# ilkyyldz95/3DmedicalImageSegmentation

Measured on AMD Instinct MI355X. Metric: training volumes/sec (96^3, 4-class), higher is better.
Workload: dtype bf16; 1 GPU; UNETR(img=96^3,patch=16,hidden=768,layers=12,heads=12,classes=4) fwd+DiceCE+bwd+AdamW, batch 2/GPU, configs[1]; global_batch=2

## Files before the change

### 3dmedicalimagesegmentation_amd/csrc/gemm_bf16.hip

```cpp
#include <type_traits>
#include "gemm_kernel.hpp"

namespace {

typedef __attribute__((address_space(3))) void lds_void_t;
typedef const __attribute__((address_space(1))) void gbl_void_t;
typedef short s16x4 __attribute__((ext_vector_type(4)));
typedef short s16x8 __attribute__((ext_vector_type(8)));
#define LDS_AS_ __attribute__((address_space(3)))

struct EpBf {
    int vec_ok;
    float* C; long ldc;
    uint16_t* Cb; long ldcb;
    const float* bias;
    const float* res; long ldr; int res_mod;
    float* pre;
    const float* aux; long ldaux;
    int act, accumulate; float alpha;
    int tc_d, tc_h, tc_w, tc_cout;
    __device__ __forceinline__ long tc_off(int m, int n) const {
        const int tap = n / tc_cout, co = n - tap * tc_cout;
        const int x = m % tc_w; int t = m / tc_w; const int y = t % tc_h; t /= tc_h; const int z = t % tc_d; const int b = t / tc_d;
        const long ov = (((long)b * 2 * tc_d + 2 * z + (tap >> 2)) * 2 * tc_h + 2 * y + ((tap >> 1) & 1)) * 2 * tc_w + 2 * x + (tap & 1);
        return ov * ldcb + co;
    }
    __device__ __forceinline__ void store(int, int m, int n, float v) const {
        v *= alpha;
        if (bias) v += bias[n];
        if (pre) pre[(long)m * ldc + n] = v;
        if (act == 1) v = gelu_fast(v);
        else if (act == 2) v *= gelu_grad_fast(aux[(long)m * ldaux + n]);
        if (res) v += res[(long)(m % res_mod) * ldr + n];
        if (C) {
            if (accumulate) v += C[(long)m * ldc + n];
            C[(long)m * ldc + n] = v;
        }
        if (Cb) {
            __bf16 h = (__bf16)v;
            Cb[tc_cout ? tc_off(m, n) : (long)m * ldcb + n] = __builtin_bit_cast(uint16_t, h);
        }
    }
    __device__ __forceinline__ void store4(int m, int n, f32x4 v) const {
        v *= alpha;
        if (bias) v += *(const f32x4*)(bias + n);
        if (pre) *(f32x4*)(pre + (long)m * ldc + n) = v;
        if (act == 1) {
#pragma unroll
            for (int e = 0; e < 4; ++e) v[e] = gelu_fast(v[e]);
        } else if (act == 2) {
            const f32x4 a = *(const f32x4*)(aux + (long)m * ldaux + n);
#pragma unroll
            for (int e = 0; e < 4; ++e) v[e] *= gelu_grad_fast(a[e]);
        }
        if (res) v += *(const f32x4*)(res + (long)(m % res_mod) * ldr + n);
        if (C) {
            if (accumulate) v += *(const f32x4*)(C + (long)m * ldc + n);
            *(f32x4*)(C + (long)m * ldc + n) = v;
        }
        if (Cb) *(bf16x4*)(Cb + (tc_cout ? tc_off(m, n) : (long)m * ldcb + n)) = __builtin_convertvector(v, bf16x4);
    }
    struct Ops { f32x4 b, a, r, c; };
    __device__ __forceinline__ Ops load4(int m, int n) const {
        Ops o;
        const f32x4 z = {0.f, 0.f, 0.f, 0.f};
        o.b = bias ? *(const f32x4*)(bias + n) : z;
        o.a = act == 2 ? *(const f32x4*)(aux + (long)m * ldaux + n) : z;
        o.r = res ? *(const f32x4*)(res + (long)(m % res_mod) * ldr + n) : z;
        o.c = (C && accumulate) ? *(const f32x4*)(C + (long)m * ldc + n) : z;
        return o;
    }
    __device__ __forceinline__ void finish4(int m, int n, f32x4 v, const Ops& o) const {
        v *= alpha;
        if (bias) v += o.b;
        if (pre) *(f32x4*)(pre + (long)m * ldc + n) = v;
        if (act == 1) {
#pragma unroll
            for (int e = 0; e < 4; ++e) v[e] = gelu_fast(v[e]);
        } else if (act == 2) {
#pragma unroll
            for (int e = 0; e < 4; ++e) v[e] *= gelu_grad_fast(o.a[e]);
        }
        if (res) v += o.r;
        if (C) {
            if (accumulate) v += o.c;
            *(f32x4*)(C + (long)m * ldc + n) = v;
        }
        if (Cb) *(bf16x4*)(Cb + (tc_cout ? tc_off(m, n) : (long)m * ldcb + n)) = __builtin_convertvector(v, bf16x4);
    }
};

template <int CPR> __device__ __forceinline__ int bkn_x(int r) {
    if constexpr (CPR >= 16) return ((r & 3) | (((r >> 3) & 1) << 2)) << 1;
    else return (((r >> 1) & 1) | (((r >> 3) & 1) << 1)) << 1;
}

__device__ __forceinline__ bool tile_of(int L, int mt, int nt, int& tm, int& tn) {
    const int T = mt * nt, per = (T + 7) >> 3;
    const int t = (L & 7) * per + (L >> 3);
    if ((L >> 3) >= per || t >= T) return false;
    tm = t % mt; tn = t / mt;
    return true;
}

template <int WM, int WN, int WVM, int WVN, bool BKN, int NS, int X3 = 0>
__global__ void __launch_bounds__(64 * WVM * WVN)
gemm_bf16_kernel(int M, int N, int K, int mt, int nt, int splits, int kper,
                 const typename std::conditional<X3 != 0, float, uint16_t>::type* __restrict__ A, long lda,
                 const typename std::conditional<X3 != 0, float, uint16_t>::type* __restrict__ B, long ldb, EpBf ep,
                 float* __restrict__ ws) {
    typedef typename std::conditional<X3 != 0, float, uint16_t>::type ET;
    constexpr int ESZ = sizeof(ET), CE = 16 / ESZ;
    constexpr int NT = 64 * WVM * WVN, BM = 16 * WM * WVM, BN = 16 * WN * WVN, BK = 128 / ESZ;
    constexpr int A_BYTES = BM * 128;
    constexpr int B_BYTES = BKN ? BK * BN * ESZ : BN * 128;
    static_assert(!(X3 != 0 && BKN) || BN >= 64, "the [K,N] fp32 image needs >= 16 chunks per row for its swizzle");
    constexpr int STAGE = A_BYTES + B_BYTES;
    constexpr int AIT = A_BYTES / 16 / NT, BIT = B_BYTES / 16 / NT;
    static_assert(A_BYTES % (16 * NT) == 0 && B_BYTES % (16 * NT) == 0, "tile must divide into whole wave DMAs");
    constexpr int G = AIT + BIT;
    static_assert(NS >= 2 && (NS - 2) * G <= 63, "vmcnt is a 6-bit counter");
    __shared__ __attribute__((aligned(1024))) char lds[NS * STAGE];

    int tm, tn;
    if (!tile_of(blockIdx.x, mt, nt, tm, tn)) return;
    const int m0 = tm * BM, n0 = tn * BN;
    const int split = blockIdx.y, kbeg = split * kper, kend = min(K, kbeg + kper);
    const int nk = (kend - kbeg) / BK;
    const int tid = threadIdx.x, lane = tid & 63;
    const int wave = __builtin_amdgcn_readfirstlane(tid >> 6), wm = wave / WVN, wn = wave % WVN;

    const ET* asrc[AIT];
    const ET* bsrc[BIT];
#pragma unroll
    for (int i = 0; i < AIT; ++i) {
        const int id = tid + i * NT, r = id >> 3, c = (id & 7) ^ ((r >> 1) & 7);
        asrc[i] = A + (long)min(m0 + r, M - 1) * lda + kbeg + c * CE;
    }
#pragma unroll
    for (int i = 0; i < BIT; ++i) {
        const int id = tid + i * NT;
        if constexpr (!BKN) {
            const int r = id >> 3, c = (id & 7) ^ ((r >> 1) & 7);
            bsrc[i] = B + (long)min(n0 + r, N - 1) * ldb + kbeg + c * CE;
        } else {
            constexpr int CPR = BN / CE;
            const int r = id / CPR, s = id % CPR;
            const int c = X3 != 0 ? (s ^ (((r >> 2) & 3) << 2)) : (s ^ bkn_x<CPR>(r));
            bsrc[i] = B + (long)(kbeg + r) * ldb + min(n0 + c * CE, N - CE);
        }
    }
    auto issue = [&](int kt, int buf) {
        char* la = lds + buf * STAGE;
        char* lb = la + A_BYTES;
#pragma unroll
        for (int i = 0; i < AIT; ++i)
            __builtin_amdgcn_global_load_lds((gbl_void_t*)(asrc[i] + (long)kt * BK), (lds_void_t*)(la + (wave * 64 + i * NT) * 16), 16, 0, 0);
#pragma unroll
        for (int i = 0; i < BIT; ++i) {
            const ET* g = BKN ? bsrc[i] + (long)kt * BK * ldb : bsrc[i] + (long)kt * BK;
            __builtin_amdgcn_global_load_lds((gbl_void_t*)g, (lds_void_t*)(lb + (wave * 64 + i * NT) * 16), 16, 0, 0);
        }
    };

    f32x4 acc[WM][WN];
#pragma unroll
    for (int i = 0; i < WM; ++i)
#pragma unroll
        for (int j = 0; j < WN; ++j) acc[i][j] = (f32x4){0.f, 0.f, 0.f, 0.f};

#pragma unroll
    for (int s = 0; s < NS - 1; ++s)
        if (s < nk) issue(s, s);
    for (int kt = 0; kt < nk; ++kt) {
        if (kt + NS - 2 < nk) asm volatile("s_waitcnt vmcnt(%0) lgkmcnt(0)\n\ts_barrier" ::"n"((NS - 2) * G) : "memory");
        else asm volatile("s_waitcnt vmcnt(0) lgkmcnt(0)\n\ts_barrier" ::: "memory");
        if (kt + NS - 1 < nk) issue(kt + NS - 1, (kt + NS - 1) % NS);
        const char* la = lds + (kt % NS) * STAGE;
        const char* lb = la + A_BYTES;
        u32x4 a[2][WM], b[2][WN];
#pragma unroll
        for (int kb = 0; kb < 2; ++kb) {
#pragma unroll
            for (int i = 0; i < WM; ++i)
                a[kb][i] = *(const u32x4*)(la + lds_tile_off((wm * WM + i) * 16 + (lane & 15), kb * 4 + (lane >> 4)));
#pragma unroll
            for (int j = 0; j < WN; ++j) {
                if constexpr (!BKN) {
                    b[kb][j] = *(const u32x4*)(lb + lds_tile_off((wn * WN + j) * 16 + (lane & 15), kb * 4 + (lane >> 4)));
                } else if constexpr (X3 != 0) {
                    const int col = (wn * WN + j) * 16 + (lane & 15), g = lane >> 4;
                    const char* pb = lb + (kb * 16 + 4 * g) * (BN * 4) + ((((col >> 2) ^ (g << 2))) << 4) + (col & 3) * 4;
#pragma unroll
                    for (int t = 0; t < 4; ++t) b[kb][j][t] = *(const uint32_t*)(pb + t * (BN * 4));
                } else {
                    constexpr int CPR = BN / 8;
                    const int cc = lane & 15, g = lane >> 4, q = cc >> 2, p = cc & 3;
                    const int r0 = kb * 32 + 8 * g + q, r1 = r0 + 4;
                    const int ch = (wn * WN + j) * 2 + (p >> 1);
                    const int s0 = ch ^ bkn_x<CPR>(r0);
                    const int s1 = ch ^ bkn_x<CPR>(r1);
                    s16x4 lo = __builtin_amdgcn_ds_read_tr16_b64_v4i16((LDS_AS_ s16x4*)(lb + r0 * (BN * 2) + s0 * 16 + (p & 1) * 8));
                    s16x4 hi = __builtin_amdgcn_ds_read_tr16_b64_v4i16((LDS_AS_ s16x4*)(lb + r1 * (BN * 2) + s1 * 16 + (p & 1) * 8));
                    s16x8 v = {lo[0], lo[1], lo[2], lo[3], hi[0], hi[1], hi[2], hi[3]};
                    b[kb][j] = __builtin_bit_cast(u32x4, v);
                }
            }
        }
        __builtin_amdgcn_sched_barrier(0);
#pragma unroll
        for (int kb = 0; kb < 2; ++kb) {
            if constexpr (X3 == 2) {
                u32x4 ah[WM], al[WM];
#pragma unroll
                for (int i = 0; i < WM; ++i) x3_dup(a[kb][i], ah[i], al[i]);
#pragma unroll
                for (int i = 0; i < WM; ++i)
#pragma unroll
                    for (int j = 0; j < WN; ++j) {
                        PrecBF16::mma(acc[i][j], b[kb][j], ah[i]);
                        PrecBF16::mma(acc[i][j], b[kb][j], al[i]);
                    }
            } else if constexpr (X3 == 1) {
                u32x4 bh[WN], bl[WN];
#pragma unroll
                for (int i = 0; i < WM; ++i) a[kb][i] = x3_words(a[kb][i]);
#pragma unroll
                for (int j = 0; j < WN; ++j) x3_dup(b[kb][j], bh[j], bl[j]);
#pragma unroll
                for (int i = 0; i < WM; ++i)
#pragma unroll
                    for (int j = 0; j < WN; ++j) {
                        PrecBF16::mma(acc[i][j], bh[j], a[kb][i]);
                        PrecBF16::mma(acc[i][j], bl[j], a[kb][i]);
                    }
            } else {
#pragma unroll
                for (int i = 0; i < WM; ++i)
#pragma unroll
                    for (int j = 0; j < WN; ++j) PrecBF16::mma(acc[i][j], b[kb][j], a[kb][i]);
            }
        }
        __builtin_amdgcn_sched_barrier(0);
    }

    const bool vec4 = ep.vec_ok;
    if (vec4 && splits == 1) {
        constexpr int RB = WM * WN <= 4 ? WM : 1;
#pragma unroll
        for (int i0 = 0; i0 < WM; i0 += RB) {
            EpBf::Ops ops[RB][WN];
#pragma unroll
            for (int i = 0; i < RB; ++i)
#pragma unroll
                for (int j = 0; j < WN; ++j) {
                    const int m = min(m0 + (wm * WM + i0 + i) * 16 + (lane & 15), M - 1);
                    const int n = min(n0 + (wn * WN + j) * 16 + 4 * (lane >> 4), N - 4);
                    ops[i][j] = ep.load4(m, n);
                }
#pragma unroll
            for (int i = 0; i < RB; ++i)
#pragma unroll
                for (int j = 0; j < WN; ++j) {
                    const int m = m0 + (wm * WM + i0 + i) * 16 + (lane & 15);
                    const int n = n0 + (wn * WN + j) * 16 + 4 * (lane >> 4);
                    if (m < M && n < N) ep.finish4(m, n, acc[i0 + i][j], ops[i][j]);
                }
        }
        return;
    }
#pragma unroll
    for (int i = 0; i < WM; ++i)
#pragma unroll
        for (int j = 0; j < WN; ++j) {
            const int m = m0 + (wm * WM + i) * 16 + (lane & 15);
            const int n = n0 + (wn * WN + j) * 16 + 4 * (lane >> 4);
            if (m >= M || n >= N) continue;
            if (vec4) {
                if (splits > 1) *(f32x4*)(ws + ((long)split * M + m) * N + n) = acc[i][j];
                else ep.store4(m, n, acc[i][j]);
            } else {
#pragma unroll
                for (int r = 0; r < 4; ++r)
                    if (n + r < N) {
                        if (splits > 1) ws[((long)split * M + m) * N + n + r] = acc[i][j][r];
                        else ep.store(0, m, n + r, acc[i][j][r]);
                    }
            }
        }
}

template <int WM, int WN, int WVM, int WVN, bool BKN, int NS, int X3 = 0>
int launch_bf16(int M, int N, int K, const typename std::conditional<X3 != 0, float, uint16_t>::type* A, long lda,
                const typename std::conditional<X3 != 0, float, uint16_t>::type* B, long ldb, const EpBf& ep,
                float* ws, size_t ws_bytes, hipStream_t st, int* partial_splits = nullptr) {
    constexpr int BM = 16 * WM * WVM, BN = 16 * WN * WVN, BKE = X3 != 0 ? 32 : 64;
    const int mt = cdiv(M, BM), nt = cdiv(N, BN), ksteps = K / BKE;
    const long tiles = (long)mt * nt;
    int splits = 1;
    const int min_steps = X3 != 0 ? 48 : 24;
    if (tiles < 192 && ksteps >= min_steps) splits = std::min(ksteps / (min_steps / 2), (int)((512 + tiles - 1) / tiles));
    if (const char* e = getenv("UNETR_GEMM_SPLITS")) { int v = atoi(e); if (v > 0) splits = std::min(v, ksteps); }
    while (splits > 1 && (size_t)splits * M * N * sizeof(float) > ws_bytes) --splits;
    if (splits < 1 || ws == nullptr) splits = 1;
    const int kper = cdiv(ksteps, splits) * BKE;
    splits = cdiv(K, kper);
    const int per = cdiv(tiles, 8);
    hipLaunchKernelGGL((gemm_bf16_kernel<WM, WN, WVM, WVN, BKN, NS, X3>), dim3(per * 8, splits), dim3(64 * WVM * WVN), 0, st,
                       M, N, K, mt, nt, splits, kper, A, lda, B, ldb, ep, ws);
    if (partial_splits) *partial_splits = splits;
    if (splits > 1 && !partial_splits)
        hipLaunchKernelGGL((splitk_reduce_kernel<EpBf, false>), dim3(cdiv(N, 64), cdiv(M, 4), 1), dim3(256), 0, st, M, N, splits, ws, ep);
    return unetr_check_launch();
}

template <int BUF>
struct BufC { static constexpr int value = BUF; };

template <int WN>
__device__ __forceinline__ void big_epilogue(f32x4 (&acc)[8][WN], const EpBf& ep, char* lds, int M, int N, int m0, int n0,
                                             int wave, int lane, int wr, int wc) {
    const int mb = m0 + wr * 128 + (lane & 15), nb = n0 + wc * (16 * WN) + 4 * (lane >> 4);
    if (!ep.vec_ok) {
        for (int t = 0; t < 8 * WN; ++t) {
            const int i = t / WN, j = t - i * WN, m = mb + i * 16, n = nb + j * 16;
            f32x4 v = (f32x4){0.f, 0.f, 0.f, 0.f};
#pragma clang loop unroll(full)
            for (int ii = 0; ii < 8; ++ii)
#pragma clang loop unroll(full)
                for (int jj = 0; jj < WN; ++jj) v = (ii == i && jj == j) ? acc[ii][jj] : v;
            if (m < M)
                for (int r = 0; r < 4; ++r)
                    if (n + r < N) ep.store(0, m, n + r, v[r]);
        }
        return;
    }
    const int kind = (ep.act == 1 ? 1 : ep.act == 2 ? 2 : 0);
    char* const stg = lds + wave * 16384;
    const int rr = lane >> 4, rc = lane & 15;
    const int ncol = n0 + wc * (16 * WN) + rc * 4;
    const bool cok = rc < 4 * WN && ncol < N;
    f32x4 bias4 = (f32x4){0.f, 0.f, 0.f, 0.f};
    if (ep.bias && cok) bias4 = *(const f32x4*)(ep.bias + ncol);
    auto half = [&](auto kc, auto hc) __attribute__((always_inline)) {
        constexpr int KIND = decltype(kc)::value, h = decltype(hc)::value;
#pragma clang loop unroll(full)
        for (int i = 0; i < 4; ++i)
#pragma clang loop unroll(full)
            for (int j = 0; j < WN; ++j) {
                const int r = i * 16 + (lane & 15), ch = j * 4 + (lane >> 4);
                *(f32x4*)(stg + r * 256 + ((ch ^ (r & 7)) << 4)) = acc[h * 4 + i][j] * ep.alpha;
            }
        asm volatile("s_waitcnt lgkmcnt(0)" ::: "memory");
#pragma clang loop unroll(full)
        for (int it = 0; it < 16; ++it) {
            const int r = it * 4 + rr, m = m0 + wr * 128 + h * 64 + r;
            f32x4 v = *(const f32x4*)(stg + r * 256 + ((rc ^ (r & 7)) << 4)) + bias4;
            if (m < M && cok) {
                if (ep.pre) *(f32x4*)(ep.pre + (long)m * ep.ldc + ncol) = v;
                if constexpr (KIND == 1) {
#pragma unroll
                    for (int e = 0; e < 4; ++e) v[e] = gelu_fast(v[e]);
                } else if constexpr (KIND == 2) {
                    const f32x4 a = *(const f32x4*)(ep.aux + (long)m * ep.ldaux + ncol);
#pragma unroll
                    for (int e = 0; e < 4; ++e) v[e] *= gelu_grad_fast(a[e]);
                }
                if (ep.res) v += *(const f32x4*)(ep.res + (long)(m % ep.res_mod) * ep.ldr + ncol);
                if (ep.C) {
                    if (ep.accumulate) v += *(const f32x4*)(ep.C + (long)m * ep.ldc + ncol);
                    *(f32x4*)(ep.C + (long)m * ep.ldc + ncol) = v;
                }
                if (ep.Cb) *(bf16x4*)(ep.Cb + (long)m * ep.ldcb + ncol) = __builtin_convertvector(v, bf16x4);
            }
        }
        asm volatile("s_waitcnt lgkmcnt(0)" ::: "memory");
    };
    if (kind == 1) { half(BufC<1>{}, BufC<0>{}); half(BufC<1>{}, BufC<1>{}); }
    else if (kind == 2) { half(BufC<2>{}, BufC<0>{}); half(BufC<2>{}, BufC<1>{}); }
    else { half(BufC<0>{}, BufC<0>{}); half(BufC<0>{}, BufC<1>{}); }
}

template <int WN>
__global__ void __launch_bounds__(512, 2)
gemm_bf16_big_kernel(int M, int N, int K, int mt, int nt, int n_fast,
                     const uint16_t* __restrict__ A, long lda, const uint16_t* __restrict__ B, long ldb, EpBf ep) {
    constexpr int NT = 512, HALF = 128 * 128, BN = 64 * WN, BUFB = 2 * HALF + BN * 128;
    constexpr int LDSB = 2 * BUFB > 8 * 16384 ? 2 * BUFB : 8 * 16384;
    __shared__ __attribute__((aligned(1024))) char lds[LDSB];

    int tm, tn;
    {
        const int T = mt * nt, per = (T + 7) >> 3, L = blockIdx.x;
        const int t = (L & 7) * per + (L >> 3);
        if ((L >> 3) >= per || t >= T) return;
        if (n_fast) { tn = t % nt; tm = t / nt; } else { tm = t % mt; tn = t / mt; }
    }
    const int m0 = tm * 256, n0 = tn * BN;
    const int nk = K / 64;
    const int tid = threadIdx.x, lane = tid & 63;
    const int wave = __builtin_amdgcn_readfirstlane(tid >> 6), wr = wave >> 2, wc = wave & 3;

    const uint16_t* asrc[2][2];
    const uint16_t* bsrc[WN];
#pragma unroll
    for (int h = 0; h < 2; ++h)
#pragma unroll
        for (int i = 0; i < 2; ++i) {
            const int id = tid + i * NT, r = id >> 3, c = (id & 7) ^ ((r >> 1) & 7);
            asrc[h][i] = A + (long)min(m0 + h * 128 + r, M - 1) * lda + c * 8;
        }
#pragma unroll
    for (int i = 0; i < WN; ++i) {
        const int id = tid + i * NT, r = id >> 3, c = (id & 7) ^ ((r >> 1) & 7);
        bsrc[i] = B + (long)min(n0 + r, N - 1) * ldb + c * 8;
    }
    auto dma = [&](const uint16_t* const (&src)[2], int T, char* dst) __attribute__((always_inline)) {
#pragma unroll
        for (int i = 0; i < 2; ++i)
            __builtin_amdgcn_global_load_lds((gbl_void_t*)(src[i] + (long)T * 64), (lds_void_t*)(dst + (wave * 64 + i * NT) * 16), 16, 0, 0);
    };
    auto dmab = [&](int T, char* dst) __attribute__((always_inline)) {
#pragma unroll
        for (int i = 0; i < WN; ++i)
            __builtin_amdgcn_global_load_lds((gbl_void_t*)(bsrc[i] + (long)T * 64), (lds_void_t*)(dst + (wave * 64 + i * NT) * 16), 16, 0, 0);
    };
    int off[2];
#pragma unroll
    for (int kh = 0; kh < 2; ++kh) off[kh] = lds_tile_off(lane & 15, kh * 4 + (lane >> 4));

    f32x4 acc[8][WN];
#pragma unroll
    for (int i = 0; i < 8; ++i)
#pragma unroll
        for (int j = 0; j < WN; ++j) acc[i][j] = (f32x4){0.f, 0.f, 0.f, 0.f};
    u32x4 af[4][2], bf[WN][2];
    dma(asrc[0], 0, lds);
    dma(asrc[1], 0, lds + HALF);
    dmab(0, lds + 2 * HALF);
    if (nk > 1) {
        dmab(1, lds + BUFB + 2 * HALF);
        asm volatile("s_waitcnt vmcnt(%0)\n\ts_barrier" ::"n"(WN) : "memory");
    } else {
        asm volatile("s_waitcnt vmcnt(0)\n\ts_barrier" ::: "memory");
    }
    if (wr == 1) asm volatile("s_barrier" ::: "memory");
    __builtin_amdgcn_sched_barrier(0);

#define BIG_MEM_END() do { asm volatile("s_waitcnt lgkmcnt(0)\n\ts_barrier" ::: "memory"); __builtin_amdgcn_sched_barrier(0); } while (0)
#define BIG_CMP_END(last_) do { __builtin_amdgcn_sched_barrier(0); if (!(last_)) asm volatile("s_barrier" ::: "memory"); __builtin_amdgcn_sched_barrier(0); } while (0)
#define BIG_HALF(qa_) do {                                                                           \
        __builtin_amdgcn_s_setprio(1);                                                               \
        _Pragma("unroll") for (int kh = 0; kh < 2; ++kh)                                             \
            _Pragma("unroll") for (int i = 0; i < 4; ++i)                                            \
                _Pragma("unroll") for (int j = 0; j < WN; ++j)                                       \
                    PrecBF16::mma(acc[(qa_) * 4 + i][j], bf[j][kh], af[i][kh]);                      \
        __builtin_amdgcn_s_setprio(0);                                                               \
    } while (0)

    auto ktile = [&](int T, auto bufc) __attribute__((always_inline)) {
        constexpr int b = decltype(bufc)::value;
        char* const cur = lds + b * BUFB;
        char* const oth = lds + (b ^ 1) * BUFB;
        const char* la = cur + wr * HALF;
        const char* lb = cur + 2 * HALF + wc * (16 * WN) * 128;
        const bool n1 = T + 1 < nk, n2 = T + 2 < nk;
        {
#pragma unroll
            for (int kh = 0; kh < 2; ++kh) {
#pragma unroll
                for (int j = 0; j < WN; ++j) bf[j][kh] = *(const u32x4*)(lb + off[kh] + j * 2048);
            }
            __builtin_amdgcn_sched_barrier(0);
#pragma unroll
            for (int kh = 0; kh < 2; ++kh) {
#pragma unroll
                for (int i = 0; i < 4; ++i) af[i][kh] = *(const u32x4*)(la + off[kh] + i * 2048);
            }
            if (n1) { dma(asrc[0], T + 1, oth); dma(asrc[1], T + 1, oth + HALF); }
            BIG_MEM_END();
            BIG_HALF(0);
            BIG_CMP_END(false);
#pragma unroll
            for (int kh = 0; kh < 2; ++kh) {
#pragma unroll
                for (int i = 0; i < 4; ++i) af[i][kh] = *(const u32x4*)(la + off[kh] + (4 + i) * 2048);
            }
            if (n2) {
                dmab(T + 2, cur + 2 * HALF);
                asm volatile("s_waitcnt vmcnt(%0)" ::"n"(WN) : "memory");
            } else if (n1) {
                asm volatile("s_waitcnt vmcnt(0)" ::: "memory");
            }
            BIG_MEM_END();
            BIG_HALF(1);
            BIG_CMP_END(!n1 && wr == 1);
        }
    };
    for (int T = 0; T < nk; T += 2) {
        ktile(T, BufC<0>{});
        if (T + 1 < nk) ktile(T + 1, BufC<1>{});
    }
#undef BIG_MEM_END
#undef BIG_CMP_END
#undef BIG_HALF

    big_epilogue<WN>(acc, ep, lds, M, N, m0, n0, wave, lane, wr, wc);
}

static int launch_bf16_big(int M, int N, int K, const uint16_t* A, long lda, const uint16_t* B, long ldb, const EpBf& ep, hipStream_t st, int wn) {
    const int BN = 64 * wn;
    const int mt = cdiv(M, 256), nt = cdiv(N, BN);
    const long tiles = (long)mt * nt;
    const long cost_m = (long)M * std::min(8, nt) + N, cost_n = M + (long)N * std::min(8, mt);
    const int n_fast = cost_n < cost_m;
    const int per = cdiv(tiles, 8);
#define BIG_GO(W_) hipLaunchKernelGGL(gemm_bf16_big_kernel<W_>, dim3(per * 8), dim3(512), 0, st, M, N, K, mt, nt, n_fast, A, lda, B, ldb, ep)
    if (wn == 2) BIG_GO(2); else if (wn == 3) BIG_GO(3); else BIG_GO(4);
#undef BIG_GO
    return unetr_check_launch();
}

static int big_tile_width(int M, int N, int K) {
    if (const char* e = getenv("UNETR_GEMM_BIG_WN")) { const int v = atoi(e); if (v >= 2 && v <= 4) return v; }
    int best = 0; double best_t = 1e30;
    for (int wn = 4; wn >= 2; --wn) {
        const long tiles = (long)cdiv(M, 256) * cdiv(N, 64 * wn);
        if (tiles < 128) continue;
        if (wn == 2 && K < 2048) continue;
        const double t = (double)cdiv(tiles, 256) * (wn + 1.5);
        if (t < best_t - 1e-9) { best_t = t; best = wn; }
    }
    return best;
}

#ifndef GW_WAVES
#define GW_WAVES 4
#endif
constexpr int GW_MAX = 64;
struct GwProblem { const uint16_t* dy; const uint16_t* x; float* dw; int M, N, K, tile0, ntn, step_idx; };
struct GwFuse { float* pb; const float* gb; float* mb; float* vb; uint16_t* sb; const float* steps; float lr, b1, b2, eps, wd; uint32_t* sw; };
struct GwArgs { int n; GwFuse f; GwProblem p[GW_MAX]; };

template <int NS, int BKT, int FUSE>
__global__ void __launch_bounds__(256, GW_WAVES)
gemm_bf16_grouped_wgrad_kernel(GwArgs ga) {
    constexpr int BT = 128;
    constexpr int IMG = BKT * BT * 2, STAGE = 2 * IMG, PCS = IMG / 16 / 256, G = 2 * PCS, CPR = 16;
    __shared__ __attribute__((aligned(1024))) char lds[NS * STAGE];
    int pi = 0;
    const int t = blockIdx.x;
    for (int hi_ = ga.n - 1; pi < hi_;) {
        const int mid = (pi + hi_ + 1) >> 1;
        if (t >= ga.p[mid].tile0) pi = mid; else hi_ = mid - 1;
    }
    const GwProblem& pr = ga.p[pi];
    const int lt = t - pr.tile0, tn = lt % pr.ntn, tk = lt / pr.ntn;
    const int n0 = tn * BT, k0 = tk * BT, M = pr.M;
    const int nk = (M + BKT - 1) / BKT;
    const int tid = threadIdx.x, lane = tid & 63;
    const int wave = __builtin_amdgcn_readfirstlane(tid >> 6), wm = wave >> 1, wn = wave & 1;

    int prow[PCS], acol[PCS], bcol[PCS];
#pragma unroll
    for (int i = 0; i < PCS; ++i) {
        const int id = tid + i * 256, r = id / CPR, sl = id % CPR, c = sl ^ bkn_x<CPR>(r);
        prow[i] = r;
        acol[i] = min(n0 + c * 8, pr.N - 8);
        bcol[i] = min(k0 + c * 8, pr.K - 8);
    }
    auto issue = [&](int kt, int buf) {
        char* la = lds + buf * STAGE;
        char* lb = la + IMG;
#pragma unroll
        for (int i = 0; i < PCS; ++i) {
            const long row = min(kt * BKT + prow[i], M - 1);
            __builtin_amdgcn_global_load_lds((gbl_void_t*)(pr.dy + row * pr.N + acol[i]), (lds_void_t*)(la + (wave * 64 + i * 256) * 16), 16, 0, 0);
        }
#pragma unroll
        for (int i = 0; i < PCS; ++i) {
            const long row = min(kt * BKT + prow[i], M - 1);
            __builtin_amdgcn_global_load_lds((gbl_void_t*)(pr.x + row * pr.K + bcol[i]), (lds_void_t*)(lb + (wave * 64 + i * 256) * 16), 16, 0, 0);
        }
    };
    f32x4 acc[4][4];
#pragma unroll
    for (int i = 0; i < 4; ++i)
#pragma unroll
        for (int j = 0; j < 4; ++j) acc[i][j] = (f32x4){0.f, 0.f, 0.f, 0.f};

#pragma unroll
    for (int s = 0; s < NS - 1; ++s)
        if (s < nk) issue(s, s);
    const int cc = lane & 15, g = lane >> 4, q = cc >> 2, p = cc & 3;
    for (int kt = 0; kt < nk; ++kt) {
        if (kt + NS - 2 < nk) asm volatile("s_waitcnt vmcnt(%0) lgkmcnt(0)\n\ts_barrier" ::"n"((NS - 2) * G) : "memory");
        else asm volatile("s_waitcnt vmcnt(0) lgkmcnt(0)\n\ts_barrier" ::: "memory");
        if (kt + NS - 1 < nk) issue(kt + NS - 1, (kt + NS - 1) % NS);
        const char* la = lds + (kt % NS) * STAGE;
        const char* lb = la + IMG;
#pragma unroll
        for (int kb = 0; kb < BKT / 32; ++kb) {
            const int r0 = kb * 32 + 8 * g + q, r1 = r0 + 4;
            const int x0s = bkn_x<CPR>(r0), x1s = bkn_x<CPR>(r1);
            const bool live = kt * BKT + kb * 32 + 8 * g < M;
            u32x4 a[4], b[4];
#pragma unroll
            for (int i = 0; i < 4; ++i) {
                const int ch = (wm * 4 + i) * 2 + (p >> 1);
                s16x4 lo = __builtin_amdgcn_ds_read_tr16_b64_v4i16((LDS_AS_ s16x4*)(la + r0 * (BT * 2) + (ch ^ x0s) * 16 + (p & 1) * 8));
                s16x4 hi = __builtin_amdgcn_ds_read_tr16_b64_v4i16((LDS_AS_ s16x4*)(la + r1 * (BT * 2) + (ch ^ x1s) * 16 + (p & 1) * 8));
                s16x8 v = {lo[0], lo[1], lo[2], lo[3], hi[0], hi[1], hi[2], hi[3]};
                const u32x4 w = __builtin_bit_cast(u32x4, v);
                a[i] = live ? w : (u32x4){0u, 0u, 0u, 0u};
            }
#pragma unroll
            for (int j = 0; j < 4; ++j) {
                const int ch = (wn * 4 + j) * 2 + (p >> 1);
                s16x4 lo = __builtin_amdgcn_ds_read_tr16_b64_v4i16((LDS_AS_ s16x4*)(lb + r0 * (BT * 2) + (ch ^ x0s) * 16 + (p & 1) * 8));
                s16x4 hi = __builtin_amdgcn_ds_read_tr16_b64_v4i16((LDS_AS_ s16x4*)(lb + r1 * (BT * 2) + (ch ^ x1s) * 16 + (p & 1) * 8));
                s16x8 v = {lo[0], lo[1], lo[2], lo[3], hi[0], hi[1], hi[2], hi[3]};
                b[j] = __builtin_bit_cast(u32x4, v);
            }
#pragma unroll
            for (int i = 0; i < 4; ++i)
#pragma unroll
                for (int j = 0; j < 4; ++j) PrecBF16::mma(acc[i][j], b[j], a[i]);
        }
    }
    static_assert(NS * STAGE >= 4 * 8192, "8 KB of staging per wave");
    __syncthreads();
    char* stg = lds + wave * 8192;
    const int rr = lane >> 4, rc = lane & 15;
    const int kcol = k0 + wn * 64 + rc * 4;
    [[maybe_unused]] AdamWCoef c{};
    [[maybe_unused]] long off0 = 0;
    if constexpr (FUSE == 1) {
        c = adamw_coef(ga.f.lr, ga.f.b1, ga.f.b2, ga.f.eps, ga.f.wd, ga.f.steps[pr.step_idx]);
        off0 = pr.dw - ga.f.gb;
    }
#pragma unroll
    for (int h = 0; h < 2; ++h) {
#pragma unroll
        for (int ii = 0; ii < 2; ++ii)
#pragma unroll
            for (int j = 0; j < 4; ++j) {
                const int r = ii * 16 + cc;
                *(f32x4*)(stg + r * 256 + (((j * 4 + g) ^ (r & 15)) << 4)) = acc[2 * h + ii][j];
            }
        asm volatile("s_waitcnt lgkmcnt(0)" ::: "memory");
        if constexpr (FUSE == 2) {
            const long offg = pr.dw - ga.f.gb;
#pragma unroll
            for (int it = 0; it < 8; ++it) {
                const int r = it * 4 + rr, n = n0 + wm * 64 + h * 32 + r;
                const f32x4 gv = *(const f32x4*)(stg + r * 256 + ((rc ^ (r & 15)) << 4));
                if (n < pr.N && kcol < pr.K) *(bf16x4*)(ga.f.sb + offg + (long)n * pr.K + kcol) = __builtin_convertvector(gv, bf16x4);
            }
        } else if constexpr (FUSE == 0) {
#pragma unroll
            for (int it = 0; it < 8; ++it) {
                const int r = it * 4 + rr, n = n0 + wm * 64 + h * 32 + r;
                const f32x4 gv = *(const f32x4*)(stg + r * 256 + ((rc ^ (r & 15)) << 4));
                if (n < pr.N && kcol < pr.K) __builtin_nontemporal_store(gv, (f32x4*)(pr.dw + (long)n * pr.K + kcol));
            }
        } else {
            const GwFuse& f = ga.f;
#pragma unroll 2
            for (int it = 0; it < 8; it += 2) {
                f32x4 gv[2], pv[2], mv[2], vv[2];
                long idx[2];
                bool ok[2];
#pragma unroll
                for (int u = 0; u < 2; ++u) {
                    const int r = (it + u) * 4 + rr, n = n0 + wm * 64 + h * 32 + r;
                    ok[u] = n < pr.N && kcol < pr.K;
                    idx[u] = off0 + (long)n * pr.K + kcol;
                    gv[u] = *(const f32x4*)(stg + r * 256 + ((rc ^ (r & 15)) << 4));
                    if (ok[u]) {
                        pv[u] = __builtin_nontemporal_load((const f32x4*)(f.pb + idx[u]));
                        mv[u] = __builtin_nontemporal_load((const f32x4*)(f.mb + idx[u]));
                        vv[u] = __builtin_nontemporal_load((const f32x4*)(f.vb + idx[u]));
                    }
                }
#pragma unroll
                for (int u = 0; u < 2; ++u) {
                    if (!ok[u]) continue;
#pragma unroll
                    for (int e = 0; e < 4; ++e) {
                        float pe = pv[u][e], me = mv[u][e], ve = vv[u][e];
                        adamw_elem(pe, me, ve, gv[u][e], c);
                        pv[u][e] = pe; mv[u][e] = me; vv[u][e] = ve;
                    }
                    __builtin_nontemporal_store(pv[u], (f32x4*)(f.pb + idx[u]));
                    __builtin_nontemporal_store(mv[u], (f32x4*)(f.mb + idx[u]));
                    __builtin_nontemporal_store(vv[u], (f32x4*)(f.vb + idx[u]));
                    if (f.sb) *(bf16x4*)(f.sb + idx[u]) = __builtin_convertvector(pv[u], bf16x4);
                    if (f.sw) *(u32x4*)(f.sw + idx[u]) = x3_words(__builtin_bit_cast(u32x4, pv[u]));
                }
            }
        }
        if (h == 0) asm volatile("s_waitcnt lgkmcnt(0)" ::: "memory");
    }
}

__global__ void __launch_bounds__(256) cast_bf16_kernel(const float* __restrict__ src, uint16_t* __restrict__ dst, long n8) {
    for (long i = blockIdx.x * 256L + threadIdx.x; i < n8; i += (long)gridDim.x * 256) {
        const f32x4 a = ((const f32x4*)src)[2 * i], b = ((const f32x4*)src)[2 * i + 1];
        float v[8] = {a[0], a[1], a[2], a[3], b[0], b[1], b[2], b[3]};
        ((u32x4*)dst)[i] = PrecBF16::pack(v);
    }
}

__global__ void __launch_bounds__(256) add_cast_bf16_kernel(const float* __restrict__ a, const float* __restrict__ b, float* __restrict__ out,
                                                            uint16_t* __restrict__ out16, long n4) {
    for (long i = blockIdx.x * 256L + threadIdx.x; i < n4; i += (long)gridDim.x * 256) {
        const f32x4 v = ((const f32x4*)a)[i] + ((const f32x4*)b)[i];
        ((f32x4*)out)[i] = v;
        if (out16) ((bf16x4*)out16)[i] = __builtin_convertvector(v, bf16x4);
    }
}

__global__ void __launch_bounds__(256) split_stack_kernel(const float* __restrict__ src, uint16_t* __restrict__ dst, long n8, long plane, int second) {
    for (long i = blockIdx.x * 256L + threadIdx.x; i < n8; i += (long)gridDim.x * 256) {
        const f32x4 a = ((const f32x4*)src)[2 * i], b = ((const f32x4*)src)[2 * i + 1];
        float v[8] = {a[0], a[1], a[2], a[3], b[0], b[1], b[2], b[3]}, r[8];
        const u32x4 hi = PrecBF16::pack(v);
#pragma unroll
        for (int e = 0; e < 4; ++e) {
            r[2 * e] = v[2 * e] - __builtin_bit_cast(float, hi[e] << 16);
            r[2 * e + 1] = v[2 * e + 1] - __builtin_bit_cast(float, hi[e] & 0xffff0000u);
        }
        const u32x4 lo = PrecBF16::pack(r);
        ((u32x4*)dst)[i] = hi;
        ((u32x4*)(dst + plane))[i] = second ? lo : hi;
        ((u32x4*)(dst + 2 * plane))[i] = second ? hi : lo;
    }
}

constexpr int SS_MAX = 64;
struct SsProblem { const float* src; uint16_t* dst; long n8; int second; int blk0; int nblk; };
struct SsArgs { int n; SsProblem p[SS_MAX]; };
__global__ void __launch_bounds__(256) split_stack_grouped_kernel(SsArgs a) {
    int pi = 0, hi_ = a.n - 1;
    while (pi < hi_) {
        const int mid = (pi + hi_ + 1) >> 1;
        if ((int)blockIdx.x >= a.p[mid].blk0) pi = mid; else hi_ = mid - 1;
    }
    const SsProblem& pr = a.p[pi];
    const float* __restrict__ src = pr.src;
    uint16_t* __restrict__ dst = pr.dst;
    const long n8 = pr.n8, plane = n8 * 8;
    const int second = pr.second;
    for (long i = ((long)blockIdx.x - pr.blk0) * 256L + threadIdx.x; i < n8; i += (long)pr.nblk * 256) {
        const f32x4 x = ((const f32x4*)src)[2 * i], y = ((const f32x4*)src)[2 * i + 1];
        float v[8] = {x[0], x[1], x[2], x[3], y[0], y[1], y[2], y[3]}, r[8];
        const u32x4 hi = PrecBF16::pack(v);
#pragma unroll
        for (int e = 0; e < 4; ++e) {
            r[2 * e] = v[2 * e] - __builtin_bit_cast(float, hi[e] << 16);
            r[2 * e + 1] = v[2 * e + 1] - __builtin_bit_cast(float, hi[e] & 0xffff0000u);
        }
        const u32x4 lo = PrecBF16::pack(r);
        ((u32x4*)dst)[i] = hi;
        ((u32x4*)(dst + plane))[i] = second ? lo : hi;
        ((u32x4*)(dst + 2 * plane))[i] = second ? hi : lo;
    }
}

__global__ void __launch_bounds__(256) cast_bf16_tail_kernel(const float* __restrict__ src, uint16_t* __restrict__ dst, long beg, long n) {
    const long i = beg + blockIdx.x * 256L + threadIdx.x;
    if (i < n) { __bf16 h = (__bf16)src[i]; dst[i] = __builtin_bit_cast(uint16_t, h); }
}

}

static int gemm_bf16_impl(const unetr_gemm_bf16_desc* d, const void* A, const void* B, float* C, void* Cb,
                          float* ws, size_t ws_bytes, void* stream, int* psp) {
    if (!d || !A || !B || (!C && !Cb)) return UNETR_ERR_ARG;
    if (d->x3) {
        if (Cb || !C || d->tc_cout > 0 || (d->x3 != 1 && d->x3 != 2)) return UNETR_ERR_ARG;
        return unetr_gemm_x3_dma(d, (const float*)A, (const float*)B, d->x3 == 2, C, ws, ws_bytes, stream, psp);
    }
    const int M = d->M, N = d->N, K = d->K;
    if (M <= 0 || N <= 0 || K <= 0) return UNETR_ERR_ARG;
    if (K % 64 || d->lda % 8 || d->ldb % 8 || ((uintptr_t)A & 15) || ((uintptr_t)B & 15)) return UNETR_ERR_UNSUPPORTED;
    if (d->b_kn && (N % 8 || N < 8)) return UNETR_ERR_UNSUPPORTED;
    if (d->act == 2 && !d->aux) return UNETR_ERR_ARG;
    if (d->accumulate && !C) return UNETR_ERR_ARG;
    hipStream_t st = (hipStream_t)stream;
    auto al16 = [](const void* p) { return ((uintptr_t)p & 15) == 0; };
    const int vec_ok = (N % 4 == 0) && (!C || (d->ldc % 4 == 0 && al16(C))) && (!Cb || (d->ldcb % 4 == 0 && ((uintptr_t)Cb & 7) == 0)) &&
                       (!d->bias || al16(d->bias)) && (!d->res || (d->ldr % 4 == 0 && al16(d->res))) && (!d->pre || al16(d->pre)) &&
                       (!d->aux || (d->ldaux % 4 == 0 && al16(d->aux))) && al16(ws);
    if (d->tc_cout > 0 && (C || !Cb || d->pre || d->accumulate || d->tc_cout % 4 || N != 8 * d->tc_cout || d->tc_d <= 0 || d->tc_h <= 0 ||
                           d->tc_w <= 0 || M % (d->tc_d * d->tc_h * d->tc_w))) return UNETR_ERR_UNSUPPORTED;
    EpBf ep{vec_ok, C, d->ldc, (uint16_t*)Cb, d->ldcb, d->bias, d->res, d->ldr, d->res_mod > 0 ? d->res_mod : M,
            d->pre, d->aux, d->ldaux, d->act, d->accumulate, d->alpha, d->tc_d, d->tc_h, d->tc_w, d->tc_cout > 0 ? d->tc_cout : 0};
    const uint16_t* a = (const uint16_t*)A;
    const uint16_t* b = (const uint16_t*)B;
    const int env_cfg = getenv("UNETR_GEMM_CFG") ? atoi(getenv("UNETR_GEMM_CFG")) : 0;
    const bool few128 = K <= 512 && (long)cdiv(M, 128) * cdiv(N, 128) < 128;
    const bool big = env_cfg == 128 || (env_cfg == 0 && M >= 1024 && N >= 128 && !few128);
    if (!d->b_kn && d->tc_cout <= 0 && (env_cfg == 256 || (env_cfg == 0 && M >= 1024))) {
        const int wn = env_cfg == 256 ? (getenv("UNETR_GEMM_BIG_WN") ? big_tile_width(M, N, K) : 4) : big_tile_width(M, N, K);
        if (wn) return launch_bf16_big(M, N, K, a, d->lda, b, d->ldb, ep, st, wn);
    }
#define BF16_GO(WM_, WN_, BKN_, NS_) return launch_bf16<WM_, WN_, 2, 2, BKN_, NS_>(M, N, K, a, d->lda, b, d->ldb, ep, ws, ws_bytes, st, psp)
    int cfg = env_cfg;
    if (!big && (cfg == 0 || cfg == 64)) {
        cfg = 6464;
        if (env_cfg == 0 && K <= 1024 && N <= 1024) cfg = d->b_kn ? 3264 : 6432;
        if (env_cfg == 0 && K <= 1024 && d->b_kn && N > 1024 && N % 64 == 0) cfg = 3264;
        if (env_cfg == 0 && M > 512) {
            if (!d->b_kn) {
                if (N >= 3072 || (N >= 2304 && M >= 960)) cfg = 6496;
                else if (K >= 2048 && N <= 1024) cfg = 6432;
            } else if (N % 128 == 0) {
                if ((K >= 2048 && N <= 1024) || (K <= 1024 && N > 1024)) cfg = 64128;
            }
        }
    }
    if (!d->b_kn) {
        if (big) BF16_GO(4, 4, false, 2);
        if (cfg == 6432) BF16_GO(2, 1, false, 4);
        if (cfg == 3264) BF16_GO(1, 2, false, 4);
        if (cfg == 64128) BF16_GO(2, 4, false, 3);
        if (cfg == 6496) BF16_GO(2, 3, false, 3);
        BF16_GO(2, 2, false, 4);
    }
    if (big) BF16_GO(4, 4, true, 2);
    if (cfg == 3264) BF16_GO(1, 2, true, 4);
    if (cfg == 64128) BF16_GO(2, 4, true, 3);
    BF16_GO(2, 2, true, 4);
#undef BF16_GO
}

int unetr_gemm_x3_dma(const unetr_gemm_bf16_desc* d, const float* A, const float* B, int b_words, float* C, float* ws, size_t ws_bytes, void* stream,
                      int* psp) {
    const int M = d->M, N = d->N, K = d->K;
    if (M <= 0 || N <= 0 || K <= 0) return UNETR_ERR_ARG;
    if (K % 32 || d->lda % 4 || d->ldb % 4 || ((uintptr_t)A & 15) || ((uintptr_t)B & 15) || N % 4) return UNETR_ERR_UNSUPPORTED;
    if (d->b_kn && N < 64) return UNETR_ERR_UNSUPPORTED;
    auto al16 = [](const void* p) { return ((uintptr_t)p & 15) == 0; };
    const int vec_ok = (d->ldc % 4 == 0 && al16(C)) && (!d->bias || al16(d->bias)) && (!d->res || (d->ldr % 4 == 0 && al16(d->res))) &&
                       (!d->pre || al16(d->pre)) && (!d->aux || (d->ldaux % 4 == 0 && al16(d->aux))) && al16(ws);
    if (!vec_ok) return UNETR_ERR_UNSUPPORTED;
    EpBf ep{1, C, d->ldc, nullptr, 0, d->bias, d->res, d->ldr, d->res_mod > 0 ? d->res_mod : M, d->pre, d->aux, d->ldaux, d->act,
            d->accumulate, d->alpha, 0, 0, 0, 0};
    hipStream_t st = (hipStream_t)stream;
#define X3_GO(WM_, WN_, BKN_, NS_) do { if (b_words) return launch_bf16<WM_, WN_, 2, 2, BKN_, NS_, 2>(M, N, K, A, d->lda, B, d->ldb, ep, ws, ws_bytes, st, psp); \
                                        return launch_bf16<WM_, WN_, 2, 2, BKN_, NS_, 1>(M, N, K, A, d->lda, B, d->ldb, ep, ws, ws_bytes, st, psp); } while (0)
    if (M >= 1024 && N >= 128) { if (d->b_kn) X3_GO(4, 4, true, 2); X3_GO(4, 4, false, 2); }
    if (!d->b_kn) {
        if (K <= 1024 && N <= 1024) X3_GO(2, 1, false, 4);
        X3_GO(2, 2, false, 4);
    }
    if (K <= 1024 && N % 64 == 0) X3_GO(1, 2, true, 4);
    X3_GO(2, 2, true, 4);
#undef X3_GO
}

extern "C" int unetr_gemm_bf16(const unetr_gemm_bf16_desc* d, const void* A, const void* B, float* C, void* Cb,
                               float* ws, size_t ws_bytes, void* stream) {
    return gemm_bf16_impl(d, A, B, C, Cb, ws, ws_bytes, stream, nullptr);
}

extern "C" int unetr_gemm_bf16_ln_bwd_pf(const unetr_gemm_bf16_desc* d, const void* A, const void* B, float* C,
                                         const float* x, const float* gamma, const float* mean, const float* rstd,
                                         float* dx, void* dx_bf16, const float* dres, float* dgamma, float* dbeta,
                                         float* ln_ws, size_t ln_ws_bytes, float* ws, size_t ws_bytes, void* stream, const unetr_prefetch* pf) {
    if (!d || !C) return UNETR_ERR_ARG;
    if (d->bias || d->res || d->pre || d->act || d->accumulate || d->alpha != 1.f || d->ldc != d->N) return UNETR_ERR_UNSUPPORTED;
    int splits = 1;
    if (int e = gemm_bf16_impl(d, A, B, C, nullptr, ws, ws_bytes, stream, &splits)) return e;
    const float* dy = splits > 1 ? ws : C;
    return unetr_layernorm_bwd_partials(dy, splits, (long)d->M * d->N, x, gamma, mean, rstd, dx, dx_bf16, dres, dgamma, dbeta,
                                        d->M, d->N, ln_ws, ln_ws_bytes, stream, pf);
}

extern "C" int unetr_gemm_bf16_ln_bwd(const unetr_gemm_bf16_desc* d, const void* A, const void* B, float* C,
                                      const float* x, const float* gamma, const float* mean, const float* rstd,
                                      float* dx, void* dx_bf16, const float* dres, float* dgamma, float* dbeta,
                                      float* ln_ws, size_t ln_ws_bytes, float* ws, size_t ws_bytes, void* stream) {
    return unetr_gemm_bf16_ln_bwd_pf(d, A, B, C, x, gamma, mean, rstd, dx, dx_bf16, dres, dgamma, dbeta, ln_ws, ln_ws_bytes, ws, ws_bytes, stream, nullptr);
}

extern "C" int unetr_gemm_bf16_ln_fwd_pf(const unetr_gemm_bf16_desc* d, const void* A, const void* B, float* C,
                                         const float* gamma, const float* beta, float eps, float* y, void* y_bf16, float* mean, float* rstd,
                                         float* ws, size_t ws_bytes, void* stream, const unetr_prefetch* pf) {
    if (!d || !C) return UNETR_ERR_ARG;
    if (d->pre || d->act || d->accumulate || d->alpha != 1.f || d->ldc != d->N) return UNETR_ERR_UNSUPPORTED;
    int splits = 1;
    if (int e = gemm_bf16_impl(d, A, B, C, nullptr, ws, ws_bytes, stream, &splits)) return e;
    if (splits > 1)
        return unetr_layernorm_fwd_partials(ws, splits, (long)d->M * d->N, d->bias, d->res, d->ldr, d->res_mod > 0 ? d->res_mod : d->M,
                                            C, gamma, beta, y, y_bf16, mean, rstd, d->M, d->N, eps, stream, pf);
    return unetr_layernorm_fwd_pf(C, gamma, beta, y, y_bf16, mean, rstd, d->M, d->N, eps, stream, pf);
}

extern "C" int unetr_gemm_bf16_ln_fwd(const unetr_gemm_bf16_desc* d, const void* A, const void* B, float* C,
                                      const float* gamma, const float* beta, float eps, float* y, void* y_bf16, float* mean, float* rstd,
                                      float* ws, size_t ws_bytes, void* stream) {
    return unetr_gemm_bf16_ln_fwd_pf(d, A, B, C, gamma, beta, eps, y, y_bf16, mean, rstd, ws, ws_bytes, stream, nullptr);
}

extern "C" int unetr_cast_bf16(const float* src, void* dst, long n, void* stream) {
    if (!src || !dst || n < 0) return UNETR_ERR_ARG;
    if (n == 0) return UNETR_OK;
    hipStream_t st = (hipStream_t)stream;
    const bool al = (((uintptr_t)src & 15) | ((uintptr_t)dst & 15)) == 0;
    const long n8 = al ? n / 8 : 0;
    if (n8) hipLaunchKernelGGL(cast_bf16_kernel, dim3((unsigned)std::min<long>(cdiv(n8, 256), 4096)), dim3(256), 0, st, src, (uint16_t*)dst, n8);
    if (n8 * 8 < n) hipLaunchKernelGGL(cast_bf16_tail_kernel, dim3(cdiv(n - n8 * 8, 256)), dim3(256), 0, st, src, (uint16_t*)dst, n8 * 8, n);
    return unetr_check_launch();
}

__global__ void __launch_bounds__(256) split_words_kernel(const float* __restrict__ src, uint32_t* __restrict__ dst, long n4) {
    for (long i = blockIdx.x * 256L + threadIdx.x; i < n4; i += (long)gridDim.x * 256) ((u32x4*)dst)[i] = x3_words(((const u32x4*)src)[i]);
}

extern "C" int unetr_split_words(const float* src, void* dst, long n, void* stream) {
    if (!src || !dst || n <= 0) return UNETR_ERR_ARG;
    if ((n & 3) || (((uintptr_t)src | (uintptr_t)dst) & 15)) return UNETR_ERR_UNSUPPORTED;
    hipLaunchKernelGGL(split_words_kernel, dim3((unsigned)std::min<long>(cdiv(n / 4, 256), 8192)), dim3(256), 0, (hipStream_t)stream, src, (uint32_t*)dst, n / 4);
    return unetr_check_launch();
}

extern "C" int unetr_split_stack_bf16(const float* src, void* dst, long rows, long cols, int second, void* stream) {
    if (!src || !dst || rows <= 0 || cols <= 0) return UNETR_ERR_ARG;
    const long n = rows * cols;
    if ((n & 7) || (((uintptr_t)src | (uintptr_t)dst) & 15)) return UNETR_ERR_UNSUPPORTED;
    hipLaunchKernelGGL(split_stack_kernel, dim3((unsigned)std::min<long>(cdiv(n / 8, 256), 4096)), dim3(256), 0, (hipStream_t)stream, src, (uint16_t*)dst,
                       n / 8, n, second);
    return unetr_check_launch();
}

extern "C" int unetr_split_stack_bf16_grouped(const unetr_split_problem* probs, int n, void* stream) {
    if (!probs || n <= 0) return UNETR_ERR_ARG;
    for (int base = 0; base < n; base += SS_MAX) {
        SsArgs a;
        a.n = std::min(SS_MAX, n - base);
        int blocks = 0;
        for (int i = 0; i < a.n; ++i) {
            const unetr_split_problem& q = probs[base + i];
            const long ne = q.rows * q.cols;
            if (!q.src || !q.dst || q.rows <= 0 || q.cols <= 0) return UNETR_ERR_ARG;
            if ((ne & 7) || (((uintptr_t)q.src | (uintptr_t)q.dst) & 15)) return UNETR_ERR_UNSUPPORTED;
            const int nb = (int)std::min<long>(cdiv(ne / 8, 256), 1024);
            a.p[i] = SsProblem{q.src, (uint16_t*)q.dst, ne / 8, q.second, blocks, nb};
            blocks += nb;
        }
        hipLaunchKernelGGL(split_stack_grouped_kernel, dim3(blocks), dim3(256), 0, (hipStream_t)stream, a);
    }
    return unetr_check_launch();
}

__global__ void __launch_bounds__(256) cast_bf16_ranges_kernel(const float* __restrict__ src, uint16_t* __restrict__ dst,
                                                               const long* __restrict__ table, int nr) {
    int lo_r = 0, hi_r = nr - 1;
    const long blk = blockIdx.x;
    while (lo_r < hi_r) {
        const int mid = (lo_r + hi_r + 1) >> 1;
        if (table[3 * mid + 2] <= blk) lo_r = mid; else hi_r = mid - 1;
    }
    const long beg = table[3 * lo_r] + (blk - table[3 * lo_r + 2]) * 8192, end = min(table[3 * lo_r + 1], beg + 8192);
    for (long i = beg / 8 + threadIdx.x; i < end / 8; i += 256) {
        const f32x4 a = ((const f32x4*)src)[2 * i], b = ((const f32x4*)src)[2 * i + 1];
        float v[8] = {a[0], a[1], a[2], a[3], b[0], b[1], b[2], b[3]};
        ((u32x4*)dst)[i] = PrecBF16::pack(v);
    }
}

extern "C" int unetr_cast_bf16_ranges(const float* src_arena, void* dst_arena, const long* table_dev, int n_ranges, long n_blocks, void* stream) {
    if (!src_arena || !dst_arena || !table_dev || n_ranges <= 0 || n_blocks <= 0 || n_blocks > 0x7fffffffL) return UNETR_ERR_ARG;
    if (((uintptr_t)src_arena & 31) || ((uintptr_t)dst_arena & 15)) return UNETR_ERR_UNSUPPORTED;
    hipLaunchKernelGGL(cast_bf16_ranges_kernel, dim3((unsigned)n_blocks), dim3(256), 0, (hipStream_t)stream, src_arena, (uint16_t*)dst_arena,
                       table_dev, n_ranges);
    return unetr_check_launch();
}

extern "C" int unetr_add_cast_bf16(const float* a, const float* b, float* out, void* out_bf16, long n, void* stream) {
    if (!a || !b || !out || n <= 0) return UNETR_ERR_ARG;
    if ((n & 3) || (((uintptr_t)a | (uintptr_t)b | (uintptr_t)out) & 15) || ((uintptr_t)out_bf16 & 7)) return UNETR_ERR_UNSUPPORTED;
    hipLaunchKernelGGL(add_cast_bf16_kernel, dim3((unsigned)std::min<long>(cdiv(n / 4, 256), 2048)), dim3(256), 0, (hipStream_t)stream, a, b, out,
                       (uint16_t*)out_bf16, n / 4);
    return unetr_check_launch();
}

static int grouped_wgrad_bf16(const unetr_grouped_problem* probs, int n, const unetr_adamw_arena* a, const int* step_index, void* stream,
                              bool b16 = false) {
    if (!probs || n <= 0) return UNETR_ERR_ARG;
    if (b16 && (!a || !a->grad || !a->shadow_bf16 || a->total <= 0 || ((uintptr_t)a->grad & 15) || ((uintptr_t)a->shadow_bf16 & 7))) return UNETR_ERR_ARG;
    if (a && !b16 && (!a->param || !a->grad || !a->m || !a->v || !a->steps || !step_index || a->total <= 0)) return UNETR_ERR_ARG;
    if (a && !b16 && ((((uintptr_t)a->param | (uintptr_t)a->grad | (uintptr_t)a->m | (uintptr_t)a->v) & 15) || ((uintptr_t)a->shadow_bf16 & 7))) return UNETR_ERR_UNSUPPORTED;
    hipStream_t st = (hipStream_t)stream;
    for (int base = 0; base < n; base += GW_MAX) {
        GwArgs ga;
        ga.n = std::min(GW_MAX, n - base);
        ga.f = GwFuse{};
        if (a) ga.f = GwFuse{a->param, a->grad, a->m, a->v, (uint16_t*)a->shadow_bf16, a->steps, a->lr, a->beta1, a->beta2, a->eps, a->weight_decay,
                             b16 ? nullptr : (uint32_t*)a->shadow_x3};
        int tiles = 0;
        for (int i = 0; i < ga.n; ++i) {
            const unetr_grouped_problem& q = probs[base + i];
            if (!q.dy || !q.x || !q.dw || q.M <= 0 || q.N < 8 || q.K < 8) return UNETR_ERR_ARG;
            if (q.M % 8 || q.N % 8 || q.K % 8 || ((uintptr_t)q.dy & 15) || ((uintptr_t)q.x & 15) || ((uintptr_t)q.dw & 15)) return UNETR_ERR_UNSUPPORTED;
            if (a) {
                const long off = q.dw - a->grad;
                if (q.dw < a->grad || off + (long)q.N * q.K > a->total || (!b16 && step_index[base + i] < 0)) return UNETR_ERR_ARG;
            }
            GwProblem& g = ga.p[i];
            g.dy = (const uint16_t*)q.dy; g.x = (const uint16_t*)q.x; g.dw = q.dw; g.M = q.M; g.N = q.N; g.K = q.K;
            g.tile0 = tiles; g.ntn = cdiv(q.N, 128);
            g.step_idx = a && !b16 ? step_index[base + i] : 0;
            tiles += g.ntn * cdiv(q.K, 128);
        }
        if (b16) hipLaunchKernelGGL((gemm_bf16_grouped_wgrad_kernel<2, 32, 2>), dim3(tiles), dim3(256), 0, st, ga);
        else if (a) hipLaunchKernelGGL((gemm_bf16_grouped_wgrad_kernel<2, 32, 1>), dim3(tiles), dim3(256), 0, st, ga);
        else hipLaunchKernelGGL((gemm_bf16_grouped_wgrad_kernel<2, 32, 0>), dim3(tiles), dim3(256), 0, st, ga);
    }
    return unetr_check_launch();
}

extern "C" int unetr_gemm_bf16_grouped_wgrad(const unetr_grouped_problem* probs, int n, void* stream) {
    return grouped_wgrad_bf16(probs, n, nullptr, nullptr, stream);
}

extern "C" int unetr_gemm_bf16_grouped_wgrad_bf16out(const unetr_grouped_problem* probs, int n, const float* grad_arena, void* out_bf16_arena,
                                                     long total, void* stream) {
    unetr_adamw_arena a{};
    a.grad = grad_arena; a.shadow_bf16 = out_bf16_arena; a.total = total; a.shadow_x3 = nullptr;
    return grouped_wgrad_bf16(probs, n, &a, nullptr, stream, true);
}

extern "C" int unetr_gemm_bf16_grouped_wgrad_adamw(const unetr_grouped_problem* probs, int n, const unetr_adamw_arena* a,
                                                   const int* step_index, void* stream) {
    if (!a) return UNETR_ERR_ARG;
    return grouped_wgrad_bf16(probs, n, a, step_index, stream);
}
```

Baseline: 476.5 volumes/s.

## Software-pipeline AdamW state loads in fused wgrad epilogue for interior tiles

For full interior tiles in the fused wgrad+AdamW epilogue, a new path prefetches the param, m and v vectors a few rows ahead in a register ring. It uses 32-bit offsets with uniform scalars and overlaps staging of the second accumulator half with in-flight loads. The step value is loaded early and made wave-uniform with readfirstlane. The aim is to hide global-memory latency of the optimizer state reads behind the update math, at the cost of more VGPRs and possible occupancy loss.

```diff
diff --git a/3dmedicalimagesegmentation_amd/csrc/gemm_bf16.hip b/3dmedicalimagesegmentation_amd/csrc/gemm_bf16.hip
--- a/3dmedicalimagesegmentation_amd/csrc/gemm_bf16.hip
+++ b/3dmedicalimagesegmentation_amd/csrc/gemm_bf16.hip
@@ -537,10 +537,15 @@
 #ifndef GW_WAVES
 #define GW_WAVES 4
 #endif
+#ifndef GW_AHEAD
+#define GW_AHEAD 3
+#endif
 constexpr int GW_MAX = 64;
 struct GwProblem { const uint16_t* dy; const uint16_t* x; float* dw; int M, N, K, tile0, ntn, step_idx; };
 struct GwFuse { float* pb; const float* gb; float* mb; float* vb; uint16_t* sb; const float* steps; float lr, b1, b2, eps, wd; uint32_t* sw; };
 struct GwArgs { int n; GwFuse f; GwProblem p[GW_MAX]; };
+
+__device__ __forceinline__ float wave_uniform(float x) { return __builtin_bit_cast(float, __builtin_amdgcn_readfirstlane(__builtin_bit_cast(int, x))); }
 
 template <int NS, int BKT, int FUSE>
 __global__ void __launch_bounds__(256, GW_WAVES)
@@ -592,6 +597,8 @@
 #pragma unroll
     for (int s = 0; s < NS - 1; ++s)
         if (s < nk) issue(s, s);
+    [[maybe_unused]] float step = 0.f;
+    if constexpr (FUSE == 1) step = wave_uniform(ga.f.steps[pr.step_idx]);
     const int cc = lane & 15, g = lane >> 4, q = cc >> 2, p = cc & 3;
     for (int kt = 0; kt < nk; ++kt) {
         if (kt + NS - 2 < nk) asm volatile("s_waitcnt vmcnt(%0) lgkmcnt(0)\n\ts_barrier" ::"n"((NS - 2) * G) : "memory");
@@ -633,22 +640,81 @@
     char* stg = lds + wave * 8192;
     const int rr = lane >> 4, rc = lane & 15;
     const int kcol = k0 + wn * 64 + rc * 4;
+    auto stage_half = [&](int h) {
+#pragma unroll
+        for (int ii = 0; ii < 2; ++ii)
+#pragma unroll
+            for (int j = 0; j < 4; ++j) {
+                const int r = ii * 16 + cc;
+                *(f32x4*)(stg + r * 256 + (((j * 4 + g) ^ (r & 15)) << 4)) = acc[2 * h + ii][j];
+            }
+        asm volatile("s_waitcnt lgkmcnt(0)" ::: "memory");
+    };
+    stage_half(0);
     [[maybe_unused]] AdamWCoef c{};
     [[maybe_unused]] long off0 = 0;
     if constexpr (FUSE == 1) {
-        c = adamw_coef(ga.f.lr, ga.f.b1, ga.f.b2, ga.f.eps, ga.f.wd, ga.f.steps[pr.step_idx]);
+        c = adamw_coef(ga.f.lr, ga.f.b1, ga.f.b2, ga.f.eps, ga.f.wd, step);
         off0 = pr.dw - ga.f.gb;
+        c.step_size = wave_uniform(c.step_size);
+        c.inv_sqrt_bc2 = wave_uniform(c.inv_sqrt_bc2);
+        if (n0 + BT <= pr.N && k0 + BT <= pr.K && pr.K < (1 << 22)) {
+            const GwFuse& f = ga.f;
+            const long org = off0 + (long)(n0 + wm * 64) * pr.K + k0 + wn * 64;
+            char* const pw = (char*)(f.pb + org);
+            char* const mw = (char*)(f.mb + org);
+            char* const vw = (char*)(f.vb + org);
+            const uint32_t lane_off = (uint32_t)(rr * pr.K + rc * 4) * 4u;
+            const uint32_t row4 = (uint32_t)pr.K * 16u;
+            auto body = [&](auto sb_c, auto sw_c) {
+                constexpr bool SB = decltype(sb_c)::value, SW = decltype(sw_c)::value;
+                constexpr int AHEAD = GW_AHEAD, RING = AHEAD + 1;
+                f32x4 pq[RING], mq[RING], vq[RING];
+                uint32_t lo = lane_off;
+                asm volatile("" : "+v"(lo));
+                auto at = [&](int i) { return lo + (uint32_t)((i >> 3) * 8 + (i & 7)) * row4; };
+                auto fetch = [&](int i) {
+                    const uint32_t ix = at(i);
+                    pq[i % RING] = __builtin_nontemporal_load((const f32x4*)(pw + ix));
+                    mq[i % RING] = __builtin_nontemporal_load((const f32x4*)(mw + ix));
+                    vq[i % RING] = __builtin_nontemporal_load((const f32x4*)(vw + ix));
+                };
+#pragma unroll
+                for (int i = 0; i < AHEAD; ++i) fetch(i);
+#pragma unroll
+                for (int i = 0; i < 16; ++i) {
+                    if (i == 8) {
+                        asm volatile("s_waitcnt lgkmcnt(0)" ::: "memory");
+                        stage_half(1);
+                    }
+                    if (i + AHEAD < 16) fetch(i + AHEAD);
+                    __builtin_amdgcn_sched_barrier(0);
+                    const int r = (i & 7) * 4 + rr;
+                    const f32x4 gv = *(const f32x4*)(stg + r * 256 + ((rc ^ (r & 15)) << 4));
+                    f32x4 pv = pq[i % RING], mv = mq[i % RING], vv = vq[i % RING];
+#pragma unroll
+                    for (int e = 0; e < 4; ++e) {
+                        float pe = pv[e], me = mv[e], ve = vv[e];
+                        adamw_elem(pe, me, ve, gv[e], c);
+                        pv[e] = pe; mv[e] = me; vv[e] = ve;
+                    }
+                    const uint32_t ix = at(i);
+                    __builtin_nontemporal_store(pv, (f32x4*)(pw + ix));
+                    __builtin_nontemporal_store(mv, (f32x4*)(mw + ix));
+                    __builtin_nontemporal_store(vv, (f32x4*)(vw + ix));
+                    if constexpr (SB) *(bf16x4*)((char*)(f.sb + org) + (ix >> 1)) = __builtin_convertvector(pv, bf16x4);
+                    if constexpr (SW) *(u32x4*)((char*)(f.sw + org) + ix) = x3_words(__builtin_bit_cast(u32x4, pv));
+                }
+            };
+            if (f.sw) { if (f.sb) body(std::true_type{}, std::true_type{}); else body(std::false_type{}, std::true_type{}); }
+            else if (f.sb) body(std::true_type{}, std::false_type{});
+            else body(std::false_type{}, std::false_type{});
+            return;
+        }
     }
 #pragma unroll
     for (int h = 0; h < 2; ++h) {
-#pragma unroll
-        for (int ii = 0; ii < 2; ++ii)
-#pragma unroll
-            for (int j = 0; j < 4; ++j) {
-                const int r = ii * 16 + cc;
-                *(f32x4*)(stg + r * 256 + (((j * 4 + g) ^ (r & 15)) << 4)) = acc[2 * h + ii][j];
-            }
-        asm volatile("s_waitcnt lgkmcnt(0)" ::: "memory");
+        if (h) stage_half(h);
         if constexpr (FUSE == 2) {
             const long offg = pr.dw - ga.f.gb;
 #pragma unroll
```

After: 478.0 volumes/s (median of 3 runs). About the same (+0.3%).
